# yccyenchicheng/p2pvg

Hardware: NVIDIA H100
Metric: frames/sec (train step, device-timed) MovingMNIST 64x64 seq30 (higher is better)
Workload: dtype bf16

## Files before the change

p2pvg_b200/csrc/conv_gemm.cu:

```cuda
#include <cstdlib>

#include "tc_common.cuh"

namespace {

using namespace tc;

struct Geom {
  int N, H, W;
  int Ck, Cn;
  int M;
  int Ntot;
  int bh128, bn128;
  int bh64, bn64;
  int bw64;
  int imgs_per_group;
  int add_bf16;
  int bres;
  int swap;
  int ks, st, sgn;
};

__device__ __forceinline__ void pix_block(int pb, int P, int H, int W, int bh, int bn, int& n0, int& y0) {
  const int HW = H * W;
  if (HW >= P) {
    const int bpi = HW / P;
    n0 = pb / bpi;
    y0 = (pb - n0 * bpi) * bh;
  } else {
    n0 = pb * bn;
    y0 = 0;
  }
}

__device__ __forceinline__ void addend_load64(float4 (&a4)[16], const float* base, long long elem_off, bool is_bf16) {
  if (is_bf16) {
    const uint4* p = reinterpret_cast<const uint4*>(reinterpret_cast<const bf16*>(base) + elem_off);
#pragma unroll
    for (int j = 0; j < 8; j++) {
      const uint4 r = p[j];
      a4[j] = make_float4(__uint_as_float(r.x), __uint_as_float(r.y), __uint_as_float(r.z), __uint_as_float(r.w));
    }
  } else {
    const float4* p = reinterpret_cast<const float4*>(base + elem_off);
#pragma unroll
    for (int j = 0; j < 16; j++) a4[j] = p[j];
  }
}
__device__ __forceinline__ void addend_add32(float (&f)[32], const float4 (&a4)[16], int h, bool is_bf16) {
  if (is_bf16) {
#pragma unroll
    for (int j = 0; j < 4; j++) {
      const float4 r = a4[4 * h + j];
      float v[8];
      unpack16<bf16>(make_uint4(__float_as_uint(r.x), __float_as_uint(r.y), __float_as_uint(r.z), __float_as_uint(r.w)), v);
#pragma unroll
      for (int i = 0; i < 8; i++) f[8 * j + i] += v[i];
    }
  } else {
#pragma unroll
    for (int j = 0; j < 8; j++) {
      const float4 x4 = a4[8 * h + j];
      f[4 * j] += x4.x; f[4 * j + 1] += x4.y; f[4 * j + 2] += x4.z; f[4 * j + 3] += x4.w;
    }
  }
}

template <int KIND, int BN, bool STAT, bool EVAL = false>
__global__ void __launch_bounds__(NUM_THREADS, 1)
conv_gemm_kernel(const __grid_constant__ CUtensorMap tmA, const __grid_constant__ CUtensorMap tmB, void* __restrict__ Cv, int c_bf16,
                 long long ldc, Geom g, int accumulate, const float* __restrict__ bias, const float* __restrict__ addend,
                 const int* __restrict__ grp_src, float* __restrict__ partial, int kb_per_split, int splits,
                 float2* __restrict__ stat_partial, const float* __restrict__ eval_scale, const float* __restrict__ eval_shift, int act) {
  using C_ = Cfg<BN>;
  constexpr bool A_MN = (KIND == 1), B_MN = (KIND != 0);
  extern __shared__ uint8_t smem_raw[];
  const Smem sm = smem_setup<BN>(smem_raw);
  const bool bres = (KIND == 0) && (BN == 64) && g.bres != 0;

  const int warp = threadIdx.x >> 5, lane = threadIdx.x & 31;
  const int tiles_m = (g.M + BLOCK_M - 1) / BLOCK_M, tiles_n = (g.Ntot + BN - 1) / BN;
  const int tiles_mn = tiles_m * tiles_n;
  const int phases = (KIND == 2) ? 4 : 1;
  const int num_tiles = tiles_mn * splits * phases;
  const int cchunks = g.Ck / 64;
  const int nkb_total = (KIND == 0) ? g.ks * g.ks * cchunks : (KIND == 2) ? 4 * cchunks : (g.N * g.H * g.W + 63) / 64;

  if (warp >= 8) {
    regs_producer();
    if (warp == 8 && lane == 0) {
      uint32_t it = 0;
      if (bres) {
        mbar_expect_tx(sm.bres_bar, (uint32_t)(g.ks * g.ks) * 64 * 128);
        for (int tap = 0; tap < g.ks * g.ks; tap++) tma_load_2d(&tmB, sm.bres_bar, sm.ring + tap * 64 * 128, tap * 64, 0);
      }
      for (int t = blockIdx.x; t < num_tiles; t += gridDim.x) {
        const int ph = (KIND == 2) ? (t & 3) : 0;
        const int t2 = (KIND == 2) ? (t >> 2) : t;
        const int z = (splits == 1) ? 0 : t2 / tiles_mn, r = t2 - z * tiles_mn;
        const int mt = (tiles_n == 1) ? r : r / tiles_n, nt = (tiles_n == 1) ? 0 : r - mt * tiles_n;
        const int n0 = nt * BN;
        const int kb0 = z * kb_per_split, kb1 = min(kb0 + kb_per_split, nkb_total);
        int pn0 = 0, py0 = 0;
        if (KIND != 1) pix_block(mt, 128, g.H, g.W, g.bh128, g.bn128, pn0, py0);
        const int pa = ph >> 1, pb_ = ph & 1;
        int kn0 = 0, ky0 = 0, kx0 = 0;
        int t_kh = 0, t_kw = 0, t_cc = 0;
        int qc0[BN / 64], qdx[BN / 64], qdy[BN / 64];
        int mc0[2] = {0, 0}, mdx[2] = {0, 0}, mdy[2] = {0, 0};
        if (KIND == 1) {
          if (g.bw64 < g.W) {
            const int per_row = g.W / g.bw64;
            const int rowi = kb0 / per_row;
            kx0 = (kb0 - rowi * per_row) * g.bw64;
            kn0 = rowi / g.H;
            ky0 = rowi - kn0 * g.H;
          } else {
            pix_block(kb0, 64, g.H, g.W, g.bh64, g.bn64, kn0, ky0);
          }
#pragma unroll
          for (int q = 0; q < BN / 64; q++) {
            const int nb = n0 + 64 * q;
            const int tap = nb / g.Cn;
            const int kh = tap / g.ks;
            qc0[q] = nb - tap * g.Cn;
            qdx[q] = tap - kh * g.ks - 1;
            qdy[q] = kh - 1;
          }
          if (g.swap) {
#pragma unroll
            for (int q = 0; q < 2; q++) {
              const int mb = mt * BLOCK_M + 64 * q;
              int tap = mb / g.Cn;
              if (tap >= g.ks * g.ks) tap = g.ks * g.ks - 1;
              const int kh = tap / g.ks;
              mc0[q] = mb < g.M ? mb - tap * g.Cn : 0;
              mdx[q] = tap - kh * g.ks - 1;
              mdy[q] = kh - 1;
            }
          }
        }
        for (int kb = kb0; kb < kb1; kb++, it++) {
          const int s = bres ? (int)(it % BRES_STAGES) : (int)(it % C_::STAGES);
          const uint32_t par = (bres ? (it / BRES_STAGES) : (it / C_::STAGES)) & 1;
          mbar_wait(&sm.empty_bar[s], par ^ 1);
          uint8_t* sa = bres ? sm.ring + BRES_B_BYTES + s * A_STAGE_BYTES : sm.ring + s * C_::STAGE_BYTES;
          uint8_t* sb = sa + A_STAGE_BYTES;
          mbar_expect_tx(&sm.full_bar[s], bres ? A_STAGE_BYTES : C_::STAGE_BYTES);
          if (KIND == 0) {
            tma_load_4d(&tmA, &sm.full_bar[s], sa, t_cc * 64, g.sgn * (t_kw - 1), g.st * py0 + g.sgn * (t_kh - 1), pn0);
            if (!bres) tma_load_2d(&tmB, &sm.full_bar[s], sb, kb * 64, n0);
            if (++t_cc == cchunks) { t_cc = 0; if (++t_kw == g.ks) { t_kw = 0; t_kh++; } }
          } else if (KIND == 2) {
            const int tq = t_kh, c0 = t_cc * 64;
            if (++t_cc == cchunks) { t_cc = 0; t_kh++; }
            const int i = tq >> 1, j = tq & 1;
            const int dy = i == 0 ? 0 : (pa ? 1 : -1), ky = i == 0 ? pa + 1 : (pa ? 0 : 3);
            const int dx = j == 0 ? 0 : (pb_ ? 1 : -1), kx = j == 0 ? pb_ + 1 : (pb_ ? 0 : 3);
            tma_load_4d(&tmA, &sm.full_bar[s], sa, c0, dx, py0 + dy, pn0);
#pragma unroll
            for (int q = 0; q < BN / 64; q++)
              tma_load_2d(&tmB, &sm.full_bar[s], sb + q * 64 * 128, (ky * 4 + kx) * g.Cn + n0 + 64 * q, c0);
          } else {
            const int m0 = mt * BLOCK_M;
            if (g.swap) {
              tma_load_4d(&tmA, &sm.full_bar[s], sa, mc0[0], g.st * kx0 + mdx[0], g.st * ky0 + mdy[0], kn0);
              tma_load_4d(&tmA, &sm.full_bar[s], sa + 64 * 128, mc0[1], g.st * kx0 + mdx[1], g.st * ky0 + mdy[1], kn0);
#pragma unroll
              for (int q = 0; q < BN / 64; q++) tma_load_2d(&tmB, &sm.full_bar[s], sb + q * 64 * 128, n0 + 64 * q, kb * 64);
            } else {
              tma_load_2d(&tmA, &sm.full_bar[s], sa, m0, kb * 64);
              tma_load_2d(&tmA, &sm.full_bar[s], sa + 64 * 128, m0 + 64, kb * 64);
#pragma unroll
              for (int q = 0; q < BN / 64; q++)
                tma_load_4d(&tmB, &sm.full_bar[s], sb + q * 64 * 128, qc0[q], g.st * kx0 + qdx[q], g.st * ky0 + qdy[q], kn0);
            }
            if (g.bw64 < g.W) {
              kx0 += g.bw64;
              if (kx0 >= g.W) { kx0 = 0; if (++ky0 >= g.H) { ky0 = 0; kn0++; } }
            } else if (g.H * g.W >= 64) {
              ky0 += g.bh64;
              if (ky0 >= g.H) { ky0 = 0; kn0++; }
            } else {
              kn0 += g.bn64;
            }
          }
        }
      }
    }
  } else if (warp >= 4) {
    regs_worker();
    mma_loop<false, BN, A_MN, B_MN>(sm, num_tiles, tiles_mn, splits, kb_per_split, nkb_total, bres);
  } else {
    regs_worker();
    const int q = warp;
    __shared__ float bias_s[2 * BN];
    __shared__ float2 stat_s[STAT ? 2 * 4 * BN : 1];
    constexpr bool do_stat = STAT;
    __shared__ float ev_s[EVAL ? 2 * 2 * BN : 1];
    uint32_t lt = 0;
    for (int t = blockIdx.x; t < num_tiles; t += gridDim.x, lt++) {
      const int ph = (KIND == 2) ? (t & 3) : 0;
      const int t2 = (KIND == 2) ? (t >> 2) : t;
      const int z = (splits == 1) ? 0 : t2 / tiles_mn, r = t2 - z * tiles_mn;
      const int mt = (tiles_n == 1) ? r : r / tiles_n, nt = (tiles_n == 1) ? 0 : r - mt * tiles_n;
      const int n0 = nt * BN;
      const uint32_t acc = lt & 1;
      const int rt = q * 32 + lane;
      long long out_row = (long long)mt * BLOCK_M + rt;
      long long add_row = 0;
      bool row_ok = out_row < g.M;
      if (KIND == 2) {
        int pn0, py0;
        pix_block(mt, 128, g.H, g.W, g.bh128, g.bn128, pn0, py0);
        const int HW = g.H * g.W;
        int nn, yy, xx;
        if (HW >= 128) { nn = 0; yy = rt / g.W; xx = rt - yy * g.W; }
        else { nn = rt / HW; const int rem = rt - nn * HW; yy = rem / g.W; xx = rem - yy * g.W; }
        const int n = pn0 + nn, y = py0 + yy;
        row_ok = (n < g.N) && (y < g.H);
        const int oy = 2 * y + (ph >> 1), ox = 2 * xx + (ph & 1);
        out_row = ((long long)n * (2 * g.H) + oy) * (2 * g.W) + ox;
        if (addend && row_ok) {
          const int n2 = grp_src[n / g.imgs_per_group] * g.imgs_per_group + (n % g.imgs_per_group);
          add_row = ((long long)n2 * (2 * g.H) + oy) * (2 * g.W) + ox;
        }
      }
      if (KIND == 0 && addend && row_ok) {
        const int HW = g.H * g.W;
        const int n = (int)(out_row / HW);
        const int n2 = grp_src[n / g.imgs_per_group] * g.imgs_per_group + (n % g.imgs_per_group);
        add_row = (long long)n2 * HW + (out_row - (long long)n * HW);
      }
      if (EVAL) {
        stage_cols<BN>(ev_s + acc * 2 * BN, eval_scale, n0, g.Ntot);
        stage_cols<BN>(ev_s + acc * 2 * BN + BN, eval_shift, n0, g.Ntot);
        if (bias == nullptr) epi_bar_sync();
      }
      if (bias != nullptr) {
        stage_cols<BN>(bias_s + acc * BN, bias, n0, g.Ntot);
        epi_bar_sync();
      }
      const bool use_add = (KIND != 1) && addend != nullptr && row_ok;
      const long long aoff0 = add_row * g.Ntot + n0;
      const bool abf = g.add_bf16 != 0;
// ... 20 lines not shown
            continue;
          }
          if (bias) add_staged32(f, bias_s + acc * BN + c * 32);
          if (use_add) addend_add32(f, a4, h, abf);
          if (EVAL) {
            const float* sc = ev_s + acc * 2 * BN + c * 32;
#pragma unroll
            for (int j = 0; j < 32; j++) {
              float y = fmaf(f[j], sc[j], sc[BN + j]);
              if (act == P2PVG_ACT_LRELU) y = y > 0.f ? y : 0.2f * y;
              else if (act == P2PVG_ACT_TANH) y = tanhf(y);
              f[j] = y;
            }
          }
          if (STAT) {
            float s1[32], s2[32];
#pragma unroll
            for (int j = 0; j < 32; j++) {
              const float r = row_ok ? (c_bf16 ? bf16_round(f[j]) : f[j]) : 0.f;
              s1[j] = r;
              s2[j] = r * r;
            }
            const float cs = warp_colsum32(s1, lane), cq = warp_colsum32(s2, lane);
            stat_s[(acc * 4 + q) * BN + c * 32 + lane] = make_float2(cs, cq);
            if (!row_ok) continue;
          }
          if (c_bf16) store_row32<bf16, false>(reinterpret_cast<bf16*>(Cv) + out_row * ldc + nbase, f, accumulate, 32);
          else store_row32<float, false>(reinterpret_cast<float*>(Cv) + out_row * ldc + nbase, f, accumulate, 32);
        }
      }
      if (STAT) {
        epi_bar_sync();
        float2* dst = stat_partial + ((long long)mt * phases + ph) * g.Ntot + n0;
        for (int i = q * 32 + lane; i < BN; i += 128) {
          if (n0 + i >= g.Ntot) continue;
          const float2 a = stat_s[(acc * 4 + 0) * BN + i], b = stat_s[(acc * 4 + 1) * BN + i];
          const float2 c2 = stat_s[(acc * 4 + 2) * BN + i], d = stat_s[(acc * 4 + 3) * BN + i];
          dst[i] = make_float2((a.x + b.x) + (c2.x + d.x), (a.y + b.y) + (c2.y + d.y));
        }
      }
    }
  }
}

int map4d(CUtensorMap* m, const void* base, int N, int Hm, int Wm, int C, int bw, int bh, int bn, int s) {
  cuuint64_t dims[4] = {(cuuint64_t)C, (cuuint64_t)Wm, (cuuint64_t)Hm, (cuuint64_t)N};
  cuuint64_t strides[3] = {(cuuint64_t)C * 2, (cuuint64_t)Wm * C * 2, (cuuint64_t)Hm * Wm * C * 2};
  cuuint32_t box[4] = {64, (cuuint32_t)(bw * s), (cuuint32_t)(bh * s), (cuuint32_t)bn};
  cuuint32_t es[4] = {1, (cuuint32_t)s, (cuuint32_t)s, 1};
  CUresult r = driver().encode(m, CU_TENSOR_MAP_DATA_TYPE_BFLOAT16, 4, const_cast<void*>(base), dims, strides, box, es, CU_TENSOR_MAP_INTERLEAVE_NONE,
                     CU_TENSOR_MAP_SWIZZLE_128B, CU_TENSOR_MAP_L2_PROMOTION_L2_256B, CU_TENSOR_MAP_FLOAT_OOB_FILL_NONE);
  if (r != CUDA_SUCCESS) {
    p2pvg_set_error("conv_gemm: 4-D tensor map failed (%d): N=%d H=%d W=%d C=%d box=(%d,%d,%d) s=%d", (int)r, N, Hm, Wm, C, bw, bh, bn, s);
    return P2PVG_ERR_CUDA;
  }
  return P2PVG_OK;
}

bool box_for(int P, int H, int W, int& bh, int& bn) {
  const int HW = H * W;
  if (HW >= P) {
    if (P % W != 0 || (H % (P / W)) != 0) return false;
    bh = P / W;
    bn = 1;
  } else {
    if (P % HW != 0) return false;
    bh = H;
    bn = P / HW;
  }
  return bh * 2 <= 256 && W * 2 <= 256 && bn <= 256;
}

struct EvalEpi {
  const float* scale = nullptr;
  const float* shift = nullptr;
  int act = 0;
};

template <int KIND, int BN, bool STAT, bool EVAL>
int launch_t(const CUtensorMap& ta, const CUtensorMap& tb, void* C, int c_dtype, long long ldc, const Geom& g, int accumulate,
             const float* bias, const float* addend, const int* grp_src, float* partial, int splits, int kb_per_split, cudaStream_t st,
             float2* stat_partial, const EvalEpi& ev) {
  const long long tiles = (long long)cdiv(g.M, BLOCK_M) * cdiv(g.Ntot, BN) * splits * (KIND == 2 ? 4 : 1);
  return launch_persistent<conv_gemm_kernel<KIND, BN, STAT, EVAL>, BN>(tiles, st, "conv_gemm", ta, tb, C, (int)(c_dtype == P2PVG_BF16), ldc, g,
                                                                       accumulate, bias, addend, grp_src, partial, kb_per_split, splits,
                                                                       stat_partial, ev.scale, ev.shift, ev.act);
}

template <int KIND, int BN>
int launch(const CUtensorMap& ta, const CUtensorMap& tb, void* C, int c_dtype, long long ldc, const Geom& g, int accumulate,
           const float* bias, const float* addend, const int* grp_src, float* partial, int splits, int kb_per_split, cudaStream_t st,
           float2* stat_partial = nullptr, const EvalEpi& ev = EvalEpi()) {
  if (KIND != 1 && ev.scale != nullptr) return launch_t<KIND, BN, false, (KIND != 1)>(ta, tb, C, c_dtype, ldc, g, accumulate, bias, addend, grp_src, partial, splits, kb_per_split, st, nullptr, ev);
  if (KIND != 1 && stat_partial != nullptr) return launch_t<KIND, BN, (KIND != 1), false>(ta, tb, C, c_dtype, ldc, g, accumulate, bias, addend, grp_src, partial, splits, kb_per_split, st, stat_partial, ev);
  return launch_t<KIND, BN, false, false>(ta, tb, C, c_dtype, ldc, g, accumulate, bias, addend, grp_src, partial, splits, kb_per_split, st, nullptr, ev);
}

bool env_off(const char* name) {
  const char* v = getenv(name);
  return v != nullptr && v[0] == '0';
}

}

int p2pvg_conv_gemm_impl(int kind, const void* a, const void* b, long long ldb, void* c, int c_dtype, long long ldc, int N, int H, int W,
                         int Ck, int Cn, int Cm, const float* bias, const float* addend, const int* grp_src, int imgs_per_group,
                         int accumulate, void* ws, size_t ws_bytes, void* stat_partial_v, int addend_dtype, const float* eval_scale,
                         const float* eval_shift, int act, cudaStream_t st) {
  float2* stat_partial = reinterpret_cast<float2*>(stat_partial_v);
  EvalEpi ev;
  ev.scale = eval_scale; ev.shift = eval_shift; ev.act = act;
  static const bool bres_on = !env_off("P2PVG_CONV_BRES"), k1_swap_on = !env_off("P2PVG_K1_SWAP");
  P2PVG_REQUIRE(driver().encode != nullptr, P2PVG_ERR_UNSUPPORTED, "conv_gemm: cuTensorMapEncodeTiled unavailable");
  P2PVG_REQUIRE(kind >= 0 && kind <= 5, P2PVG_ERR_BAD_ARG, "conv_gemm: bad kind %d", kind);
  if (eval_scale != nullptr) {
    P2PVG_REQUIRE(kind == 0 || kind == 2, P2PVG_ERR_BAD_ARG, "conv_gemm: the eval-BatchNorm epilogue belongs to kinds 0 and 2");
    P2PVG_REQUIRE(eval_shift != nullptr, P2PVG_ERR_BAD_ARG, "conv_gemm: eval_scale without eval_shift");
    P2PVG_REQUIRE(stat_partial == nullptr, P2PVG_ERR_BAD_ARG, "conv_gemm: the eval-BatchNorm epilogue excludes fwd_stat_partial");
    P2PVG_REQUIRE(!accumulate, P2PVG_ERR_BAD_ARG, "conv_gemm: the eval-BatchNorm epilogue does not accumulate");
    P2PVG_REQUIRE(act == P2PVG_ACT_LRELU || act == P2PVG_ACT_TANH, P2PVG_ERR_BAD_ARG, "conv_gemm: eval epilogue act %d", act);
  }
  if (N <= 0) return P2PVG_OK;
  Geom g;
  g.N = N; g.H = H; g.W = W; g.Ck = Ck; g.Cn = Cn; g.imgs_per_group = imgs_per_group > 0 ? imgs_per_group : 1;
  g.add_bf16 = (addend != nullptr && addend_dtype == P2PVG_BF16) ? 1 : 0;
  g.swap = 0;
  g.bres = 0;
  g.ks = kind >= 3 ? 3 : 4; g.st = kind >= 3 ? 1 : 2; g.sgn = kind == 5 ? -1 : 1;
  const int taps = g.ks * g.ks;
  if (kind == 3 || kind == 5) kind = 0;
  if (kind == 4) kind = 1;
  g.bh128 = g.bn128 = g.bh64 = g.bn64 = 1;
  g.bw64 = W;
  bool ok;
  if (kind == 1) {
    if (W > 64 && W % 64 == 0 && W * g.st <= 256) { g.bw64 = 64; ok = true; }
    else ok = box_for(64, H, W, g.bh64, g.bn64);
  } else {
    ok = box_for(128, H, W, g.bh128, g.bn128);
  }
  ok = ok && (((uintptr_t)a | (uintptr_t)b | (uintptr_t)c) & 15) == 0;
  if (kind == 1) ok = ok && (Cn % 64 == 0) && (Cm % 8 == 0);
  else ok = ok && (Ck % 64 == 0) && (Cn % 32 == 0) && (ldb % 8 == 0);
  if (kind == 2 || addend != nullptr) ok = ok && (Cn % 64 == 0);
  if (!ok) {
    p2pvg_set_error("conv_gemm: shape not supported by the pixel-box tiling (kind=%d N=%d H=%d W=%d Ck=%d Cn=%d)", kind, N, H, W, Ck, Cn);
    return P2PVG_ERR_UNSUPPORTED;
  }
  CUtensorMap ta, tb;
  int rc;
  const long long pix = (long long)N * H * W;
  if (kind == 0) {
    g.M = (int)pix; g.Ntot = Cn;
    rc = map4d(&ta, a, N, g.st * H, g.st * W, Ck, W, g.bh128, g.bn128, g.st);
    if (rc) return rc;
    const int BN = Cn > 64 ? 128 : 64;
    rc = map2d(&tb, b, (long long)taps * Ck, Cn, ldb, BN);
    if (rc) return rc;
    const int nkb = taps * (Ck / 64);
    g.bres = (BN == 64 && Cn == 64 && Ck == 64 && taps <= 9 && bres_on) ? 1 : 0;
    if (BN == 128) return launch<0, 128>(ta, tb, c, c_dtype, ldc, g, accumulate, bias, addend, grp_src, nullptr, 1, nkb, st, stat_partial, ev);
    return launch<0, 64>(ta, tb, c, c_dtype, ldc, g, accumulate, bias, addend, grp_src, nullptr, 1, nkb, st, stat_partial, ev);
  }
  if (kind == 2) {
    g.M = (int)pix; g.Ntot = Cn;
    rc = map4d(&ta, a, N, H, W, Ck, W, g.bh128, g.bn128, 1);
    if (rc) return rc;
    rc = map2d(&tb, b, 16LL * Cn, Ck, ldb, 64);
    if (rc) return rc;
    const int nkb = 4 * (Ck / 64);
    const int BN = Cn > 64 ? 128 : 64;
    if (BN == 128) return launch<2, 128>(ta, tb, c, c_dtype, ldc, g, accumulate, bias, addend, grp_src, nullptr, 1, nkb, st, stat_partial, ev);
    return launch<2, 64>(ta, tb, c, c_dtype, ldc, g, accumulate, bias, addend, grp_src, nullptr, 1, nkb, st, stat_partial, ev);
  }
  P2PVG_REQUIRE(c_dtype == P2PVG_F32, P2PVG_ERR_BAD_ARG, "conv_gemm kind 1 writes fp32");
  P2PVG_REQUIRE(stat_partial == nullptr, P2PVG_ERR_BAD_ARG, "conv_gemm: BatchNorm statistics belong to the forward / data-gradient kinds");
  g.Ck = 64;
  const int nkb = (int)((pix + 63) / 64);
  g.swap = (Cm == 64 && k1_swap_on && nkb >= 16 && ws != nullptr && (size_t)2 * taps * Cn * Cm * sizeof(float) <= ws_bytes) ? 1 : 0;
  if (g.swap) {
    g.M = taps * Cn; g.Ntot = Cm;
    rc = map4d(&ta, b, N, g.st * H, g.st * W, Cn, g.bw64, g.bh64, g.bn64, g.st);
    if (rc) return rc;
    rc = map2d(&tb, a, Cm, pix, Cm, 64);
    if (rc) return rc;
  } else {
    g.M = Cm; g.Ntot = taps * Cn;
    rc = map2d(&ta, a, Cm, pix, Cm, 64);
    if (rc) return rc;
    rc = map4d(&tb, b, N, g.st * H, g.st * W, Cn, g.bw64, g.bh64, g.bn64, g.st);
    if (rc) return rc;
  }
  const int BN = (g.Ntot % 128 == 0) ? 128 : 64;
  const long long tiles = (long long)cdiv(g.M, BLOCK_M) * cdiv(g.Ntot, BN);
  int splits = g.swap ? 2 : 1;
  {
    double best = 1e300;
    const int maxs = nkb / 8 < 64 ? nkb / 8 : 64;
    const int smin = g.swap ? 2 : 1;
    for (int s = smin; s <= (maxs < smin ? smin : maxs); s++) {
      const int kb = cdiv(nkb, s), se = cdiv(nkb, kb);
      if (se > 1 && (ws == nullptr || (size_t)se * g.M * g.Ntot * sizeof(float) > ws_bytes)) continue;
      const long long rounds = cdiv((long long)tiles * se, driver().sms);
      double cost = (double)rounds * (kb + 8.0);
      if (se > 1) cost += (double)se * g.M * g.Ntot * 8.0 / 6.0e12 / (0.22e-6 * BN / 128);
      if (cost < best) { best = cost; splits = se; }
    }
  }
  int kbps = cdiv(nkb, splits);
  splits = cdiv(nkb, kbps);
  float* partial = splits > 1 ? reinterpret_cast<float*>(ws) : nullptr;
  if (BN == 128) rc = launch<1, 128>(ta, tb, c, c_dtype, ldc, g, accumulate, nullptr, nullptr, nullptr, partial, splits, kbps, st);
  else rc = launch<1, 64>(ta, tb, c, c_dtype, ldc, g, accumulate, nullptr, nullptr, nullptr, partial, splits, kbps, st);
  if (rc) return rc;
  if (splits > 1)
    return p2pvg_splitk_reduce(partial, splits, c, P2PVG_F32, ldc, Cm, taps * Cn, accumulate, nullptr, nullptr, 0, g.swap, st);
  P2PVG_REQUIRE(!g.swap, P2PVG_ERR_UNSUPPORTED, "conv_gemm kind 1 (swapped roles) needs the split-K workspace");
  return P2PVG_OK;
}
```

p2pvg_b200/csrc/gemm_tc.cu:

```cuda
#include "tc_common.cuh"

namespace {

using namespace tc;


template <typename TIn, int BN, bool A_MN, bool B_MN>
__global__ void __launch_bounds__(NUM_THREADS, 1)
gemm_tc_kernel(const __grid_constant__ CUtensorMap tmA, const __grid_constant__ CUtensorMap tmB, void* __restrict__ Cv,
               int c_bf16, long long ldc, int M, int N, int K, int accumulate, const float* __restrict__ bias,
               const void* __restrict__ addend, long long ldd, float* __restrict__ partial, int kb_per_split, int splits) {
  using C_ = Cfg<BN>;
  constexpr int ELEM = sizeof(TIn);
  constexpr int BLOCK_K = ROW_BYTES / ELEM;
  constexpr bool TF32 = (ELEM == 4);
  static_assert(!(TF32 && (A_MN || B_MN)), "tf32 path supports K-major operands only");
  extern __shared__ uint8_t smem_raw[];
  const Smem sm = smem_setup<BN>(smem_raw);

  const int warp = threadIdx.x >> 5, lane = threadIdx.x & 31;
  const int tiles_m = (M + BLOCK_M - 1) / BLOCK_M, tiles_n = (N + BN - 1) / BN;
  const int tiles_mn = tiles_m * tiles_n;
  const int num_tiles = tiles_mn * splits;
  const int nkb_total = (K + BLOCK_K - 1) / BLOCK_K;
// ... 28 lines not shown
            tma_load_2d(&tmB, &sm.full_bar[s], sb, k0, n0);
          }
        }
      }
    }
  } else if (warp >= 4) {
    regs_worker();
    mma_loop<TF32, BN, A_MN, B_MN>(sm, num_tiles, tiles_mn, splits, kb_per_split, nkb_total, false);
  } else {
    regs_worker();
    const bool split = (partial != nullptr);
    __shared__ float bias_s[2 * BN];
    uint32_t lt = 0;
    for (int t = blockIdx.x; t < num_tiles; t += gridDim.x, lt++) {
      const int z = (splits == 1) ? 0 : t / tiles_mn, r = t - z * tiles_mn;
      const int mt_ = (tiles_n == 1) ? r : r / tiles_n;
      const int m0 = mt_ * BLOCK_M, n0 = (r - mt_ * tiles_n) * BN;
      const uint32_t bsel = lt & 1;
      const long long m = (long long)m0 + threadIdx.x;
      const bool row_ok = m < M;
      if (bias != nullptr && !split) {
        stage_cols<BN>(bias_s + bsel * BN, bias, n0, N);
        epi_bar_sync();
      }
      mbar_wait(sm.acc_full_bar, lt & 1);
#pragma unroll 1
      for (int pr = 0; pr < BN / 64; pr++) {
#pragma unroll
        for (int h = 0; h < 2; h++) {
          const int c = pr * 2 + h;
          float f[32];
          read_chunk<BN>(sm, threadIdx.x, c, f);
          const int nbase = n0 + c * 32;
          if (!row_ok || nbase >= N) continue;
          const int ncols = N - nbase;
          if (split) {
            float* dst = partial + ((long long)z * M + m) * N + nbase;
            if (ncols >= 32 && ((reinterpret_cast<uintptr_t>(dst) & 15) == 0)) {
#pragma unroll
              for (int j = 0; j < 32; j += 4) *reinterpret_cast<float4*>(dst + j) = make_float4(f[j], f[j + 1], f[j + 2], f[j + 3]);
            } else {
#pragma unroll
              for (int j = 0; j < 32; j++)
                if (j < ncols) dst[j] = f[j];
            }
            continue;
          }
          if (bias) add_staged32(f, bias_s + bsel * BN + c * 32);
          if (c_bf16) {
            if (addend) add_row32<bf16, true>(f, reinterpret_cast<const bf16*>(addend) + m * ldd + nbase, ncols);
            store_row32<bf16, true>(reinterpret_cast<bf16*>(Cv) + m * ldc + nbase, f, accumulate, ncols);
          } else {
            if (addend) add_row32<float, true>(f, reinterpret_cast<const float*>(addend) + m * ldd + nbase, ncols);
            store_row32<float, true>(reinterpret_cast<float*>(Cv) + m * ldc + nbase, f, accumulate, ncols);
          }
        }
      }
    }
  }
}

template <typename TO>
__global__ void splitk_reduce_kernel(const float* __restrict__ partial, int splits, TO* __restrict__ C, long long ldc, int M, int N,
                                     int accumulate, const float* __restrict__ bias, const TO* __restrict__ addend, long long ldd,
                                     int transposed) {
  const long long total = (long long)M * N;
  for (long long idx = (long long)blockIdx.x * blockDim.x + threadIdx.x; idx < total; idx += (long long)gridDim.x * blockDim.x) {
    const long long m = idx / N;
    const int n = (int)(idx - m * N);
    const long long pidx = transposed ? (long long)n * M + m : idx;
    float acc = 0.f;
    for (int z = 0; z < splits; z++) acc += partial[(long long)z * total + pidx];
    if (bias) acc += bias[n];
    if (addend) acc += ld_f<TO>(&addend[m * ldd + n]);
    if (accumulate) acc += ld_f<TO>(&C[m * ldc + n]);
    st_f<TO>(&C[m * ldc + n], acc);
  }
}

template <typename TIn, int BN, bool A_MN, bool B_MN>
int launch(const CUtensorMap& ta, const CUtensorMap& tb, void* C, int c_dtype, long long ldc, int M, int N, int K, int accumulate,
           const float* bias, const void* addend, long long ldd, float* partial, int splits, int kb_per_split, cudaStream_t st) {
  const long long num_tiles = (long long)cdiv(M, BLOCK_M) * cdiv(N, BN) * splits;
  return launch_persistent<gemm_tc_kernel<TIn, BN, A_MN, B_MN>, BN>(num_tiles, st, "gemm_tc", ta, tb, C, (int)(c_dtype == P2PVG_BF16), ldc,
                                                                    M, N, K, accumulate, bias, addend, ldd, partial, kb_per_split, splits);
}

}

int p2pvg_gemm_tc_available() { return driver().encode != nullptr; }

int p2pvg_splitk_reduce(const float* partial, int splits, void* C, int c_dtype, long long ldc, int M, int N, int accumulate,
                        const float* bias, const void* addend, long long ldd, int transposed, cudaStream_t st) {
  const long long total = (long long)M * N;
  const int cap = driver().sms * 8;
  const int blocks = (int)((total + 255) / 256 > cap ? cap : (total + 255) / 256);
  if (c_dtype == P2PVG_BF16)
    splitk_reduce_kernel<bf16><<<blocks, 256, 0, st>>>(partial, splits, (bf16*)C, ldc, M, N, accumulate, bias, (const bf16*)addend, ldd,
                                                       transposed);
  else
    splitk_reduce_kernel<float><<<blocks, 256, 0, st>>>(partial, splits, (float*)C, ldc, M, N, accumulate, bias, (const float*)addend, ldd,
                                                        transposed);
  return p2pvg_check_launch("splitk_reduce");
}

int p2pvg_gemm_simt(const void*, int, int, long long, const void*, int, long long, void*, int, long long, int, int, int, int,
                    const float*, const void*, long long, void*, size_t, cudaStream_t);

static bool tc_operand_ok(const void* p, long long ld, int elem = 2) {
  return ((reinterpret_cast<uintptr_t>(p) & 15) == 0) && ((ld * elem) % 16 == 0);
}

int p2pvg_gemm_tf32(const void* A, long long lda, const void* B, long long ldb, void* C, int c_dtype, long long ldc, int M, int N,
                    int K, int accumulate, const float* bias, const void* addend, long long ldd, cudaStream_t st) {
  if (M <= 0 || N <= 0) return P2PVG_OK;
  if (!p2pvg_gemm_tc_available() || !tc_operand_ok(A, lda, 4) || !tc_operand_ok(B, ldb, 4) || K <= 0) return P2PVG_ERR_UNSUPPORTED;
  const int BN = (N > 64) ? 128 : 64;
  CUtensorMap ta, tb;
  int rc = map2d(&ta, A, K, M, lda, BLOCK_M, 4);
  if (rc) return rc;
  rc = map2d(&tb, B, K, N, ldb, BN, 4);
  if (rc) return rc;
  const int nkb = cdiv(K, 32);
  if (BN == 128) return launch<float, 128, false, false>(ta, tb, C, c_dtype, ldc, M, N, K, accumulate, bias, addend, ldd, nullptr, 1, nkb, st);
  return launch<float, 64, false, false>(ta, tb, C, c_dtype, ldc, M, N, K, accumulate, bias, addend, ldd, nullptr, 1, nkb, st);
}

int p2pvg_gemm_tc(const void* A, int a_mn, long long lda, const void* B, int b_mn, long long ldb, void* C, int c_dtype, long long ldc,
                  int M, int N, int K, int accumulate, const float* bias, const void* addend, long long ldd, void* workspace,
                  size_t ws_bytes, cudaStream_t st) {
  if (M <= 0 || N <= 0) return P2PVG_OK;
  extern int p2pvg_gemm_impl_forced();
  if (!p2pvg_gemm_tc_available() || !tc_operand_ok(A, lda) || !tc_operand_ok(B, ldb) || K <= 0) {
    if (p2pvg_gemm_impl_forced() == 2) {
      p2pvg_set_error("gemm_tc: operands not TMA-compatible (A=%p lda=%lld B=%p ldb=%lld K=%d, driver=%d)", A, lda, B, ldb, K,
                      p2pvg_gemm_tc_available());
      return P2PVG_ERR_UNSUPPORTED;
    }
    return p2pvg_gemm_simt(A, P2PVG_BF16, a_mn, lda, B, b_mn, ldb, C, c_dtype, ldc, M, N, K, accumulate, bias, addend, ldd, workspace, ws_bytes, st);
  }
  const int BN = (N > 64) ? 128 : 64;
  CUtensorMap ta, tb;
  int rc;
  constexpr int BLOCK_K = 64;
  if (a_mn) rc = map2d(&ta, A, M, K, lda, BLOCK_K);
  else rc = map2d(&ta, A, K, M, lda, BLOCK_M);
  if (rc) return rc;
  if (b_mn) rc = map2d(&tb, B, N, K, ldb, BLOCK_K);
  else rc = map2d(&tb, B, K, N, ldb, BN);
  if (rc) return rc;

  const int nkb = cdiv(K, BLOCK_K);
  const long long tiles = (long long)cdiv(M, BLOCK_M) * cdiv(N, BN);
  int splits = 1;
  if (tiles < 120 && nkb >= 16) {
    long long want = (2 * driver().sms + tiles - 1) / tiles;
    long long maxs = nkb / 8;
    splits = (int)(want < maxs ? want : maxs);
    if (splits < 1) splits = 1;
    size_t need = (size_t)splits * M * N * sizeof(float);
    while (splits > 1 && (workspace == nullptr || need > ws_bytes)) {
      splits /= 2;
      need = (size_t)splits * M * N * sizeof(float);
    }
  }
  int kb_per_split = cdiv(nkb, splits);
  splits = cdiv(nkb, kb_per_split);
// ... 21 lines not shown
```

p2pvg_b200/csrc/tc_common.cuh:

```cuda
#pragma once
#include <cuda.h>

#include "common.cuh"

namespace tc {

__device__ __forceinline__ uint32_t smem_u32(const void* p) { return (uint32_t)__cvta_generic_to_shared(p); }

__device__ __forceinline__ void mbar_init(uint64_t* bar, uint32_t count) {
  asm volatile("mbarrier.init.shared::cta.b64 [%0], %1;" ::"r"(smem_u32(bar)), "r"(count));
}
__device__ __forceinline__ void mbar_expect_tx(uint64_t* bar, uint32_t bytes) {
  asm volatile("mbarrier.arrive.expect_tx.shared::cta.b64 _, [%0], %1;" ::"r"(smem_u32(bar)), "r"(bytes) : "memory");
}
__device__ __forceinline__ void mbar_wait(uint64_t* bar, uint32_t parity) {
  asm volatile(
      "{\n\t"
      ".reg .pred P1;\n\t"
      "WAIT_LOOP:\n\t"
      "mbarrier.try_wait.parity.shared::cta.b64 P1, [%0], %1;\n\t"
      "@P1 bra DONE;\n\t"
      "bra WAIT_LOOP;\n\t"
      "DONE:\n\t"
      "}" ::"r"(smem_u32(bar)),
// ... 73 lines not shown
  return d;
}

template <bool TF32, int BN, bool A_MN, bool B_MN>
__device__ __forceinline__ void wgmma_kblock(float (&acc)[2][BN / 2], uint64_t da, uint64_t db, bool first) {
  constexpr int UMMA_K = TF32 ? 8 : 16;
  constexpr int KSTEPS = 4;
  constexpr uint32_t A_STEP = (A_MN ? UMMA_K * 128 : 32) >> 4, B_STEP = (B_MN ? UMMA_K * 128 : 32) >> 4;
#pragma unroll
  for (int k = 0; k < KSTEPS; k++) {
    const uint32_t sc = (first && k == 0) ? 0u : 1u;
#pragma unroll
    for (int h = 0; h < 2; h++) {
      const uint64_t a = da + (uint64_t)(h * (8192 >> 4) + k * A_STEP), b = db + (uint64_t)(k * B_STEP);
      if constexpr (TF32) {
        if constexpr (BN == 128) wgmma_tf32_n128(acc[h], a, b, sc);
        else wgmma_tf32_n64(acc[h], a, b, sc);
      } else {
        if constexpr (BN == 128) wgmma_bf16_n128<A_MN ? 1 : 0, B_MN ? 1 : 0>(acc[h], a, b, sc);
        else wgmma_bf16_n64<A_MN ? 1 : 0, B_MN ? 1 : 0>(acc[h], a, b, sc);
      }
    }
  }
}

template <int BN>
__device__ __forceinline__ void acc_to_smem(const float (&acc)[2][BN / 2], float* buf, int ld, int t) {
  const int w = t >> 5, l = t & 31;
#pragma unroll
  for (int h = 0; h < 2; h++) {
    float* r0 = buf + (64 * h + 16 * w + (l >> 2)) * ld + 2 * (l & 3);
#pragma unroll
    for (int j = 0; j < BN / 8; j++) {
      *reinterpret_cast<float2*>(r0 + 8 * j) = make_float2(acc[h][4 * j], acc[h][4 * j + 1]);
      *reinterpret_cast<float2*>(r0 + 8 * ld + 8 * j) = make_float2(acc[h][4 * j + 2], acc[h][4 * j + 3]);
    }
  }
}

__device__ __forceinline__ void mbar_arrive(uint64_t* bar) {
  asm volatile("mbarrier.arrive.shared::cta.b64 _, [%0];" ::"r"(smem_u32(bar)) : "memory");
}
__device__ __forceinline__ void tma_load_4d(const CUtensorMap* desc, uint64_t* bar, void* smem_dst, int c0, int c1, int c2, int c3) {
  asm volatile(
      "cp.async.bulk.tensor.4d.shared::cluster.global.mbarrier::complete_tx::bytes [%0], [%1, {%3, %4, %5, %6}], [%2];" ::"r"(
          smem_u32(smem_dst)),
      "l"(reinterpret_cast<uint64_t>(desc)), "r"(smem_u32(bar)), "r"(c0), "r"(c1), "r"(c2), "r"(c3)
      : "memory");
}

template <int OFF>
__device__ __forceinline__ void colsum_stage(float (&v)[32], int lane) {
  const bool upper = (lane & OFF) != 0;
#pragma unroll
  for (int j = 0; j < OFF; j++) {
    const float send = upper ? v[j] : v[j + OFF];
    const float keep = upper ? v[j + OFF] : v[j];
    v[j] = keep + __shfl_xor_sync(0xffffffffu, send, OFF);
  }
  if constexpr (OFF > 1) colsum_stage<OFF / 2>(v, lane);
}
__device__ __forceinline__ float warp_colsum32(float (&v)[32], int lane) {
  colsum_stage<16>(v, lane);
  return v[0];
}
__device__ __forceinline__ float bf16_round(float x) { return __bfloat162float(__float2bfloat16_rn(x)); }

constexpr int BLOCK_M = 128;
constexpr int ROW_BYTES = 128;
constexpr int A_STAGE_BYTES = BLOCK_M * ROW_BYTES;
constexpr int NUM_THREADS = 384;

template <int BN> struct Cfg {
  static constexpr int B_STAGE_BYTES = BN * ROW_BYTES;
  static constexpr int STAGE_BYTES = A_STAGE_BYTES + B_STAGE_BYTES;
  static constexpr int STAGES = (BN == 128) ? 4 : 7;
  static constexpr int ACC_LD = BN + 4;
  static constexpr int ACC_BYTES = BLOCK_M * ACC_LD * 4;
  static constexpr int SMEM_BYTES = STAGES * STAGE_BYTES + ACC_BYTES + 1024  + 512 ;
};

constexpr int BRES_B_BYTES = 9 * 64 * 128, BRES_STAGES = 6;
static_assert(BRES_B_BYTES + BRES_STAGES * A_STAGE_BYTES <= Cfg<64>::STAGES * Cfg<64>::STAGE_BYTES, "resident weights + A ring");

struct Smem {
  uint8_t* ring;
  float* accs;
  uint64_t *full_bar, *empty_bar, *acc_full_bar, *acc_empty_bar;
  uint64_t* bres_bar;
};

template <int BN>
__device__ __forceinline__ Smem smem_setup(uint8_t* smem_raw) {
  using C_ = Cfg<BN>;
  Smem s;
  s.ring = reinterpret_cast<uint8_t*>((reinterpret_cast<uintptr_t>(smem_raw) + 1023) & ~(uintptr_t)1023);
  s.accs = reinterpret_cast<float*>(s.ring + C_::STAGES * C_::STAGE_BYTES);
  s.full_bar = reinterpret_cast<uint64_t*>(s.ring + C_::STAGES * C_::STAGE_BYTES + C_::ACC_BYTES);
  s.empty_bar = s.full_bar + C_::STAGES;
  s.acc_full_bar = s.empty_bar + C_::STAGES;
  s.acc_empty_bar = s.acc_full_bar + 1;
  s.bres_bar = s.acc_empty_bar + 1;
  if (threadIdx.x == 0) {
    for (int i = 0; i < C_::STAGES; i++) {
      mbar_init(&s.full_bar[i], 1);
      mbar_init(&s.empty_bar[i], 128);
    }
    mbar_init(s.acc_full_bar, 128);
    mbar_init(s.acc_empty_bar, 4);
    mbar_init(s.bres_bar, 1);
    asm volatile("fence.mbarrier_init.release.cluster;" ::: "memory");
  }
  __syncthreads();
  return s;
}

template <bool TF32, int BN, bool A_MN, bool B_MN>
__device__ __forceinline__ void mma_loop(const Smem& sm, int num_tiles, int tiles_mn, int splits, int kb_per_split, int nkb_total,
                                         bool bres) {
  using C_ = Cfg<BN>;
  const int wt = threadIdx.x - 128;
  const uint32_t smem0 = smem_u32(sm.ring);
  const uint64_t da0 = A_MN ? make_desc(smem0, 64 * 128, 1024) : make_desc(smem0, 0, 1024);
  const uint64_t db0 = B_MN ? make_desc(smem0 + A_STAGE_BYTES, 64 * 128, 1024) : make_desc(smem0 + A_STAGE_BYTES, 0, 1024);
  uint32_t it = 0, lt = 0;
  if (bres) mbar_wait(sm.bres_bar, 0);
  const uint64_t da0r = make_desc(smem0 + BRES_B_BYTES, 0, 1024), db0r = make_desc(smem0, 0, 1024);
  float acc[2][BN / 2];
  for (int t = blockIdx.x; t < num_tiles; t += gridDim.x, lt++) {
    const int z = (splits == 1) ? 0 : t / tiles_mn;
    const int kb0 = z * kb_per_split, kb1 = min(kb0 + kb_per_split, nkb_total);
    int prev = -1;
    for (int kb = kb0; kb < kb1; kb++, it++) {
      const int s = bres ? (int)(it % BRES_STAGES) : (int)(it % C_::STAGES);
      const uint32_t par = (bres ? (it / BRES_STAGES) : (it / C_::STAGES)) & 1;
      mbar_wait(&sm.full_bar[s], par);
      const uint64_t stage_off = (uint64_t)((uint32_t)s * (uint32_t)(C_::STAGE_BYTES >> 4));
      const uint64_t a_off = bres ? (uint64_t)((uint32_t)s * (uint32_t)(A_STAGE_BYTES >> 4)) : stage_off;
      const uint64_t b_off = bres ? (uint64_t)((uint32_t)kb * (uint32_t)((64 * 128) >> 4)) : stage_off;
      fence_regs(acc[0]);
      fence_regs(acc[1]);
      wgmma_fence();
      wgmma_kblock<TF32, BN, A_MN, B_MN>(acc, (bres ? da0r : da0) + a_off, (bres ? db0r : db0) + b_off, kb == kb0);
      wgmma_commit();
      wgmma_wait<1>();
      fence_regs(acc[0]);
      fence_regs(acc[1]);
      if (prev >= 0) mbar_arrive(&sm.empty_bar[prev]);
      prev = s;
    }
    wgmma_wait<0>();
    fence_regs(acc[0]);
    fence_regs(acc[1]);
    if (prev >= 0) mbar_arrive(&sm.empty_bar[prev]);
    mbar_wait(sm.acc_empty_bar, (lt & 1) ^ 1);
    acc_to_smem<BN>(acc, sm.accs, C_::ACC_LD, wt);
    mbar_arrive(sm.acc_full_bar);
  }
}

template <int BN>
__device__ __forceinline__ void stage_cols(float* dst, const float* src, int n0, int N) {
  for (int i = threadIdx.x; i < BN; i += 128) dst[i] = (n0 + i < N) ? src[n0 + i] : 0.f;
}

template <int BN>
__device__ __forceinline__ void read_chunk(const Smem& sm, int row, int c, float (&f)[32]) {
  const float* src = sm.accs + row * Cfg<BN>::ACC_LD + c * 32;
#pragma unroll
  for (int j = 0; j < 32; j += 4) {
    const float4 x = *reinterpret_cast<const float4*>(src + j);
    f[j] = x.x; f[j + 1] = x.y; f[j + 2] = x.z; f[j + 3] = x.w;
  }
  if (c == BN / 32 - 1) {
    __syncwarp();
    if ((threadIdx.x & 31) == 0) mbar_arrive(sm.acc_empty_bar);
  }
}

__device__ __forceinline__ void add_staged32(float (&f)[32], const float* s) {
#pragma unroll
  for (int j = 0; j < 32; j += 4) {
    const float4 b4 = *reinterpret_cast<const float4*>(s + j);
    f[j] += b4.x; f[j + 1] += b4.y; f[j + 2] += b4.z; f[j + 3] += b4.w;
  }
}

template <typename T, bool TAIL>
__device__ __forceinline__ void add_row32(float (&f)[32], const T* row, int ncols) {
#pragma unroll
  for (int j = 0; j < 32; j++)
    if (!TAIL || j < ncols) f[j] += ld_f<T>(row + j);
}

template <typename T, bool TAIL>
__device__ __forceinline__ void store_row32(T* crow, float (&f)[32], int accumulate, int ncols) {
  if (accumulate) add_row32<T, TAIL>(f, crow, ncols);
  const bool vec = !TAIL || (ncols >= 32 && (reinterpret_cast<uintptr_t>(crow) & 15) == 0);
  if (vec && (reinterpret_cast<uintptr_t>(crow) & 31) == 0) {
    if constexpr (sizeof(T) == 2) {
#pragma unroll
      for (int j = 0; j < 32; j += 16)
        st_global_256(crow + j, pack_bf16x2(f[j], f[j + 1]), pack_bf16x2(f[j + 2], f[j + 3]), pack_bf16x2(f[j + 4], f[j + 5]),
                      pack_bf16x2(f[j + 6], f[j + 7]), pack_bf16x2(f[j + 8], f[j + 9]), pack_bf16x2(f[j + 10], f[j + 11]),
                      pack_bf16x2(f[j + 12], f[j + 13]), pack_bf16x2(f[j + 14], f[j + 15]));
    } else {
#pragma unroll
      for (int j = 0; j < 32; j += 8)
        st_global_256(crow + j, __float_as_uint(f[j]), __float_as_uint(f[j + 1]), __float_as_uint(f[j + 2]), __float_as_uint(f[j + 3]),
                      __float_as_uint(f[j + 4]), __float_as_uint(f[j + 5]), __float_as_uint(f[j + 6]), __float_as_uint(f[j + 7]));
    }
  } else if (vec) {
    if constexpr (sizeof(T) == 2) {
#pragma unroll
      for (int j = 0; j < 32; j += 8)
        *reinterpret_cast<uint4*>(crow + j) =
            make_uint4(pack_bf16x2(f[j], f[j + 1]), pack_bf16x2(f[j + 2], f[j + 3]), pack_bf16x2(f[j + 4], f[j + 5]), pack_bf16x2(f[j + 6], f[j + 7]));
    } else {
#pragma unroll
      for (int j = 0; j < 32; j += 4) *reinterpret_cast<float4*>(crow + j) = make_float4(f[j], f[j + 1], f[j + 2], f[j + 3]);
    }
  } else {
#pragma unroll
    for (int j = 0; j < 32; j++)
      if (j < ncols) st_f<T>(crow + j, f[j]);
  }
}

typedef CUresult (*EncodeTiledFn)(CUtensorMap*, CUtensorMapDataType, cuuint32_t, void*, const cuuint64_t*, const cuuint64_t*,
                                  const cuuint32_t*, const cuuint32_t*, CUtensorMapInterleave, CUtensorMapSwizzle,
                                  CUtensorMapL2promotion, CUtensorMapFloatOOBfill);
struct Driver {
  EncodeTiledFn encode = nullptr;
  int sms = 132;
};

inline const Driver& driver() {
  static const Driver d = [] {
    Driver r;
    int dev = 0, sms = 0;
    if (cudaGetDevice(&dev) == cudaSuccess && cudaDeviceGetAttribute(&sms, cudaDevAttrMultiProcessorCount, dev) == cudaSuccess && sms > 0)
      r.sms = sms;
    void* fn = nullptr;
    cudaDriverEntryPointQueryResult q;
    if (cudaGetDriverEntryPoint("cuTensorMapEncodeTiled", &fn, cudaEnableDefault, &q) == cudaSuccess && q == cudaDriverEntryPointSuccess)
      r.encode = reinterpret_cast<EncodeTiledFn>(fn);
    (void)cudaGetLastError();
    return r;
  }();
  return d;
}

inline int map2d(CUtensorMap* map, const void* base, long long dim0, long long dim1, long long ld, int box1, int elem = 2) {
  cuuint64_t dims[2] = {(cuuint64_t)dim0, (cuuint64_t)dim1};
  cuuint64_t strides[1] = {(cuuint64_t)ld * elem};
  cuuint32_t box[2] = {(cuuint32_t)(ROW_BYTES / elem), (cuuint32_t)box1};
  cuuint32_t estr[2] = {1, 1};
  CUresult r = driver().encode(map, elem == 2 ? CU_TENSOR_MAP_DATA_TYPE_BFLOAT16 : CU_TENSOR_MAP_DATA_TYPE_FLOAT32, 2, const_cast<void*>(base),
                               dims, strides, box, estr, CU_TENSOR_MAP_INTERLEAVE_NONE, CU_TENSOR_MAP_SWIZZLE_128B,
                               CU_TENSOR_MAP_L2_PROMOTION_L2_256B, CU_TENSOR_MAP_FLOAT_OOB_FILL_NONE);
  if (r != CUDA_SUCCESS) {
    p2pvg_set_error("cuTensorMapEncodeTiled failed (%d): base=%p dims=(%lld,%lld) ld=%lld box1=%d", (int)r, base, dim0, dim1, ld, box1);
    return P2PVG_ERR_CUDA;
  }
  return P2PVG_OK;
}

template <auto KERN, int BN, typename... Args>
int launch_persistent(long long tiles, cudaStream_t st, const char* what, Args... args) {
  static bool smem_attr_set = false;
  if (!smem_attr_set) {
    const cudaError_t e = cudaFuncSetAttribute(KERN, cudaFuncAttributeMaxDynamicSharedMemorySize, Cfg<BN>::SMEM_BYTES);
    if (e != cudaSuccess) {
      p2pvg_set_error("%s: cudaFuncSetAttribute: %s", what, cudaGetErrorString(e));
      return P2PVG_ERR_CUDA;
    }
    smem_attr_set = true;
  }
  const int sms = driver().sms;
  KERN<<<(int)(tiles < sms ? tiles : sms), NUM_THREADS, Cfg<BN>::SMEM_BYTES, st>>>(args...);
  return p2pvg_check_launch(what);
}

}
```

Measured before the change: 198,600.

## Keep per-phase transposed-conv weights resident in shared memory for kind-2 GEMM

Extends the resident-weight (bres) path to the sub-pixel transposed convolution kernel (KIND 2). The grid is rounded down to a multiple of 4 so each CTA always handles the same phase. That lets it load that phase's 4 taps x channel-chunk weights into shared memory once, instead of re-streaming B tiles every k-block. This cuts TMA traffic and per-stage bytes, at the cost of possibly dropping up to 3 CTAs. It also adds a new MN-major descriptor path for the resident B.

```diff
diff --git a/p2pvg_b200/csrc/conv_gemm.cu b/p2pvg_b200/csrc/conv_gemm.cu
--- a/p2pvg_b200/csrc/conv_gemm.cu
+++ b/p2pvg_b200/csrc/conv_gemm.cu
@@ -33,6 +33,14 @@
   }
 }
 
+__device__ __forceinline__ void phase_tap(int ph, int tq, int& dy, int& dx, int& ky, int& kx) {
+  const int pa = ph >> 1, pb = ph & 1, i = tq >> 1, j = tq & 1;
+  dy = i == 0 ? 0 : (pa ? 1 : -1);
+  ky = i == 0 ? pa + 1 : (pa ? 0 : 3);
+  dx = j == 0 ? 0 : (pb ? 1 : -1);
+  kx = j == 0 ? pb + 1 : (pb ? 0 : 3);
+}
+
 __device__ __forceinline__ void addend_load64(float4 (&a4)[16], const float* base, long long elem_off, bool is_bf16) {
   if (is_bf16) {
     const uint4* p = reinterpret_cast<const uint4*>(reinterpret_cast<const bf16*>(base) + elem_off);
@@ -76,7 +84,7 @@
   constexpr bool A_MN = (KIND == 1), B_MN = (KIND != 0);
   extern __shared__ uint8_t smem_raw[];
   const Smem sm = smem_setup<BN>(smem_raw);
-  const bool bres = (KIND == 0) && (BN == 64) && g.bres != 0;
+  const bool bres = (KIND == 0 || (KIND == 2 && (gridDim.x & 3) == 0)) && (BN == 64) && g.bres != 0;
 
   const int warp = threadIdx.x >> 5, lane = threadIdx.x & 31;
   const int tiles_m = (g.M + BLOCK_M - 1) / BLOCK_M, tiles_n = (g.Ntot + BN - 1) / BN;
@@ -90,9 +98,18 @@
     regs_producer();
     if (warp == 8 && lane == 0) {
       uint32_t it = 0;
-      if (bres) {
+      if (bres && KIND == 0) {
         mbar_expect_tx(sm.bres_bar, (uint32_t)(g.ks * g.ks) * 64 * 128);
         for (int tap = 0; tap < g.ks * g.ks; tap++) tma_load_2d(&tmB, sm.bres_bar, sm.ring + tap * 64 * 128, tap * 64, 0);
+      } else if (bres) {
+        const int ph = blockIdx.x & 3;
+        mbar_expect_tx(sm.bres_bar, (uint32_t)nkb_total * 64 * 128);
+        for (int kb = 0; kb < nkb_total; kb++) {
+          const int tq = kb / cchunks;
+          int dy, dx, ky, kx;
+          phase_tap(ph, tq, dy, dx, ky, kx);
+          tma_load_2d(&tmB, sm.bres_bar, sm.ring + kb * 64 * 128, (ky * 4 + kx) * g.Cn, (kb - tq * cchunks) * 64);
+        }
       }
       for (int t = blockIdx.x; t < num_tiles; t += gridDim.x) {
         const int ph = (KIND == 2) ? (t & 3) : 0;
@@ -103,7 +120,6 @@
         const int kb0 = z * kb_per_split, kb1 = min(kb0 + kb_per_split, nkb_total);
         int pn0 = 0, py0 = 0;
         if (KIND != 1) pix_block(mt, 128, g.H, g.W, g.bh128, g.bn128, pn0, py0);
-        const int pa = ph >> 1, pb_ = ph & 1;
         int kn0 = 0, ky0 = 0, kx0 = 0;
         int t_kh = 0, t_kw = 0, t_cc = 0;
         int qc0[BN / 64], qdx[BN / 64], qdy[BN / 64];
@@ -154,13 +170,14 @@
           } else if (KIND == 2) {
             const int tq = t_kh, c0 = t_cc * 64;
             if (++t_cc == cchunks) { t_cc = 0; t_kh++; }
-            const int i = tq >> 1, j = tq & 1;
-            const int dy = i == 0 ? 0 : (pa ? 1 : -1), ky = i == 0 ? pa + 1 : (pa ? 0 : 3);
-            const int dx = j == 0 ? 0 : (pb_ ? 1 : -1), kx = j == 0 ? pb_ + 1 : (pb_ ? 0 : 3);
+            int dy, dx, ky, kx;
+            phase_tap(ph, tq, dy, dx, ky, kx);
             tma_load_4d(&tmA, &sm.full_bar[s], sa, c0, dx, py0 + dy, pn0);
-#pragma unroll
-            for (int q = 0; q < BN / 64; q++)
-              tma_load_2d(&tmB, &sm.full_bar[s], sb + q * 64 * 128, (ky * 4 + kx) * g.Cn + n0 + 64 * q, c0);
+            if (!bres) {
+#pragma unroll
+              for (int q = 0; q < BN / 64; q++)
+                tma_load_2d(&tmB, &sm.full_bar[s], sb + q * 64 * 128, (ky * 4 + kx) * g.Cn + n0 + 64 * q, c0);
+            }
           } else {
             const int m0 = mt * BLOCK_M;
             if (g.swap) {
@@ -347,7 +364,8 @@
              const float* bias, const float* addend, const int* grp_src, float* partial, int splits, int kb_per_split, cudaStream_t st,
              float2* stat_partial, const EvalEpi& ev) {
   const long long tiles = (long long)cdiv(g.M, BLOCK_M) * cdiv(g.Ntot, BN) * splits * (KIND == 2 ? 4 : 1);
-  return launch_persistent<conv_gemm_kernel<KIND, BN, STAT, EVAL>, BN>(tiles, st, "conv_gemm", ta, tb, C, (int)(c_dtype == P2PVG_BF16), ldc, g,
+  const int grid_align = (KIND == 2 && g.bres) ? 4 : 1;
+  return launch_persistent<conv_gemm_kernel<KIND, BN, STAT, EVAL>, BN>(tiles, grid_align, st, "conv_gemm", ta, tb, C, (int)(c_dtype == P2PVG_BF16), ldc, g,
                                                                        accumulate, bias, addend, grp_src, partial, kb_per_split, splits,
                                                                        stat_partial, ev.scale, ev.shift, ev.act);
 }
@@ -435,6 +453,8 @@
     if (rc) return rc;
     const int nkb = 4 * (Ck / 64);
     const int BN = Cn > 64 ? 128 : 64;
+    const int sms = driver().sms;
+    g.bres = (Cn == 64 && Ck <= 128 && bres_on && (long long)cdiv(g.M, BLOCK_M) * 4 > sms && sms >= 4) ? 1 : 0;
     if (BN == 128) return launch<2, 128>(ta, tb, c, c_dtype, ldc, g, accumulate, bias, addend, grp_src, nullptr, 1, nkb, st, stat_partial, ev);
     return launch<2, 64>(ta, tb, c, c_dtype, ldc, g, accumulate, bias, addend, grp_src, nullptr, 1, nkb, st, stat_partial, ev);
   }
diff --git a/p2pvg_b200/csrc/gemm_tc.cu b/p2pvg_b200/csrc/gemm_tc.cu
--- a/p2pvg_b200/csrc/gemm_tc.cu
+++ b/p2pvg_b200/csrc/gemm_tc.cu
@@ -134,7 +134,7 @@
 int launch(const CUtensorMap& ta, const CUtensorMap& tb, void* C, int c_dtype, long long ldc, int M, int N, int K, int accumulate,
            const float* bias, const void* addend, long long ldd, float* partial, int splits, int kb_per_split, cudaStream_t st) {
   const long long num_tiles = (long long)cdiv(M, BLOCK_M) * cdiv(N, BN) * splits;
-  return launch_persistent<gemm_tc_kernel<TIn, BN, A_MN, B_MN>, BN>(num_tiles, st, "gemm_tc", ta, tb, C, (int)(c_dtype == P2PVG_BF16), ldc,
+  return launch_persistent<gemm_tc_kernel<TIn, BN, A_MN, B_MN>, BN>(num_tiles, 1, st, "gemm_tc", ta, tb, C, (int)(c_dtype == P2PVG_BF16), ldc,
                                                                     M, N, K, accumulate, bias, addend, ldd, partial, kb_per_split, splits);
 }
 
diff --git a/p2pvg_b200/csrc/tc_common.cuh b/p2pvg_b200/csrc/tc_common.cuh
--- a/p2pvg_b200/csrc/tc_common.cuh
+++ b/p2pvg_b200/csrc/tc_common.cuh
@@ -179,6 +179,7 @@
 
 constexpr int BRES_B_BYTES = 9 * 64 * 128, BRES_STAGES = 6;
 static_assert(BRES_B_BYTES + BRES_STAGES * A_STAGE_BYTES <= Cfg<64>::STAGES * Cfg<64>::STAGE_BYTES, "resident weights + A ring");
+static_assert(4 * 2 * 64 * 128 <= BRES_B_BYTES, "kind-2 phase weights: 4 taps x 2 channel chunks");
 
 struct Smem {
   uint8_t* ring;
@@ -222,7 +223,7 @@
   const uint64_t db0 = B_MN ? make_desc(smem0 + A_STAGE_BYTES, 64 * 128, 1024) : make_desc(smem0 + A_STAGE_BYTES, 0, 1024);
   uint32_t it = 0, lt = 0;
   if (bres) mbar_wait(sm.bres_bar, 0);
-  const uint64_t da0r = make_desc(smem0 + BRES_B_BYTES, 0, 1024), db0r = make_desc(smem0, 0, 1024);
+  const uint64_t da0r = make_desc(smem0 + BRES_B_BYTES, 0, 1024), db0r = B_MN ? make_desc(smem0, 64 * 128, 1024) : make_desc(smem0, 0, 1024);
   float acc[2][BN / 2];
   for (int t = blockIdx.x; t < num_tiles; t += gridDim.x, lt++) {
     const int z = (splits == 1) ? 0 : t / tiles_mn;
@@ -364,7 +365,7 @@
 }
 
 template <auto KERN, int BN, typename... Args>
-int launch_persistent(long long tiles, cudaStream_t st, const char* what, Args... args) {
+int launch_persistent(long long tiles, int grid_align, cudaStream_t st, const char* what, Args... args) {
   static bool smem_attr_set = false;
   if (!smem_attr_set) {
     const cudaError_t e = cudaFuncSetAttribute(KERN, cudaFuncAttributeMaxDynamicSharedMemorySize, Cfg<BN>::SMEM_BYTES);
@@ -375,7 +376,9 @@
     smem_attr_set = true;
   }
   const int sms = driver().sms;
-  KERN<<<(int)(tiles < sms ? tiles : sms), NUM_THREADS, Cfg<BN>::SMEM_BYTES, st>>>(args...);
+  int grid = (int)(tiles < sms ? tiles : sms);
+  grid -= grid % grid_align;
+  KERN<<<grid, NUM_THREADS, Cfg<BN>::SMEM_BYTES, st>>>(args...);
   return p2pvg_check_launch(what);
 }
 
```

Result: faster. 202,900, median of 6 (+2.2%).
